# yjxiong/action-detection

Hardware: AMD Instinct MI355X
Metric: proposals/sec (9-seg BNInception SSN fwd+bwd) (higher is better)
Workload: dtype f32

## Files before the change

action-detection_amd/csrc/wgrad_pl.hip:

```cpp
#include "planes.h"

#include <algorithm>
#include <cmath>
#include <cstdlib>
#include <map>
#include <mutex>
#include <vector>

namespace {

using namespace pl;

struct WgPlArgs {
    const void* g_hi;
    const void* g_lo;
    const void* x_hi;
    const void* x_lo;
    float* part;
    unsigned long long* trace;
    int dbg;
    const float* g_scale;
    const float* x_scale;
    int g_row_split, g_row_gap;
    int N, Cin, H, W;
// ... 215 lines not shown
        __builtin_amdgcn_sched_barrier(0);
        read_begin(st[1]);
        mfma(cur, ks + NSTAGE, st[0], nxt);
        ++ks;
        const uint32_t o = st[0];
#pragma unroll
        for (int i = 0; i + 1 < NSTAGE; ++i) st[i] = st[i + 1];
        st[NSTAGE - 1] = o;
    };
    trc.mark1(p);
    for (int t = 0; t < nks; t += 2) {
        half(fr0, fr1);
        half(fr1, fr0);
    }
    SSN_WAIT_LGKM0();
    SSN_WAIT_VMCNT(0);
    trc.mark2(p);

    const float inv = 1.f / (*p.g_scale * *p.x_scale);
    const int KK = p.kh * p.kw;
    float* out = p.part + (long)z * p.M * p.ldp;
#pragma unroll
    for (int j = 0; j < TC; ++j) {
        const int ci = c0 + (wc * TC + j) * 32 + li;
        if (ci >= p.Cin) continue;
#pragma unroll
        for (int i = 0; i < TM; ++i) {
#pragma unroll
            for (int r = 0; r < 16; ++r) {
                const int m = m0 + (wm * TM + i) * 32 + (r & 3) + 8 * (r >> 2) + 4 * lh;
                if (m < p.M) out[(long)m * p.ldp + ci * KK + (int)tap] = acc[i][j][r] * inv;
            }
        }
    }
    if (do_bias && li == 0) {
        const float ginv = 1.f / *p.g_scale;
#pragma unroll
        for (int i = 0; i < TM; ++i)
#pragma unroll
            for (int r = 0; r < 16; ++r) {
                const int m = m0 + (wm * TM + i) * 32 + (r & 3) + 8 * (r >> 2) + 4 * lh;
                if (m < p.M) out[(long)m * p.ldp + p.K] = accb[i][r] * ginv;
            }
    }
    trc.end(p);
}

template <int WM, int WC, int TM, int TC>
__global__ __launch_bounds__(256, (TM * TC >= 6) ? 1 : 2) void wgrad_pl_kernel(WgPlArgs p) {
    __shared__ __attribute__((aligned(1024))) uint32_t lds[wgpl_lds_dwords<WM, WC, TM, TC>()];
    wgrad_pl_body<WM, WC, TM, TC>(p, blockIdx.x, lds);
}

template <int TM, int TC, int XP>
constexpr int wgpl9_lds_bytes() {
    return 2 * ((2 * TM) * 2 * 4 * 1024 + (2 * TC) * 2 * XP * 1024);
}

template <int KK, int TM, int TC, int XP, int KG = 1, int KH = 3, int KW = 3, int PH = 1, int PW = 1>
__device__ __forceinline__ void wgrad_pl9_body(const WgPlArgs& p, const uint32_t bid, unsigned char* lds) {
    constexpr int NS = 64, KSC = NS / 16;
    constexpr int KSG = KSC / KG;
    static_assert(KK == 1 || KK == KH * KW, "1x1, or all taps of the window");
    static_assert((KSG * KK) % 2 == 0, "steps come in pairs");
    static_assert(KG == 1 || KG == 2, "one or two wave groups");
    static_assert(XP % KG == 0, "X pieces split evenly between the wave groups");
    constexpr int BM = 2 * TM * 32, BC = 2 * TC * 32;
    constexpr int FA = BM / 32, FB = BC / 32;
    constexpr int A_BYTES = FA * 2 * KSC * 1024;
    constexpr int X_BYTES = FB * 2 * XP * 1024;
    constexpr int STAGE = A_BYTES + X_BYTES;
    static_assert(2 * STAGE == wgpl9_lds_bytes<TM, TC, XP>(), "LDS size");

    const int tid = threadIdx.x;
    WgTrace trc;
    trc.begin(p);
    const int lane = tid & 63, wave8 = wave_uniform(tid >> 6);
    const int wave = wave8 & 3, grp = wave8 >> 2;
    const int wm = wave >> 1, wc = wave & 1;
    const int li = lane & 31, lh = lane >> 5;

    const uint32_t tiles = (uint32_t)p.n_mtiles * (uint32_t)p.n_ctiles;
    const uint32_t logical = xcd_remap(bid, tiles * (uint32_t)p.splits);
    uint32_t z, tile, mt, ct;
    fd_divmod(logical, p.div_tiles, z, tile);
    fd_divmod(tile, p.div_ct, mt, ct);
    const int m0 = (int)mt * BM, c0 = (int)ct * BC;
    constexpr int BH = KK > 1 ? (PH > KH - 1 - PH ? PH : KH - 1 - PH) : 0, BW = KK > 1 ? (PW > KW - 1 - PW ? PW : KW - 1 - PW) : 0;
    const int Wp = p.W + BW, SP = (p.H + BH) * Wp;
    const int D = KK > 1 ? PH * Wp + PW : 0;
    const uint32_t T = (uint32_t)p.N * (uint32_t)SP;

    const int op = wave >> 1, plane = wave & 1;
    const void *xh = p.x_hi, *xl = p.x_lo, *gh = p.g_hi, *gl = p.g_lo;
    const uint32_t xbytes = p.x_bytes, gbytes = p.g_bytes, xgrp = p.x_grp_bytes, ggrp = p.g_grp_bytes, ximg = p.x_img_bytes, gimg = p.g_img_bytes;
    const __amdgpu_buffer_rsrc_t rsrc = op ? pl_rsrc(plane ? xl : xh, xbytes) : pl_rsrc(plane ? gl : gh, gbytes);
    const uint32_t grp_bytes = op ? xgrp : ggrp;
    const uint32_t img_bytes = op ? ximg : gimg;
    const int dsl = lane >> 2;
    const uint32_t lane_grp = (uint32_t)(lane & 3) * grp_bytes;
    constexpr int NF = FA > FB ? FA : FB;
    uint32_t frag_so[NF];
#pragma unroll
    for (int f = 0; f < NF; ++f) {
        const int ch = (op ? c0 : m0) + f * 32;
        const int gap = (!op && ch >= p.g_row_split) ? p.g_row_gap : 0;
        frag_so[f] = (uint32_t)((ch + gap) / 8) * grp_bytes;
    }
    const int ck_begin = (int)z * p.ksteps_per_split;
    const int total_ck = (int)((T + NS - 1) / NS);
    int ck_end = ck_begin + p.ksteps_per_split;
    if (ck_end > total_ck) ck_end = total_ck;

    constexpr int NPMAX = (XP > KSC ? XP : KSC) / KG;
    const int npieces = wave_uniform(op ? XP / KG : KSC / KG);
    const int lane_slot0 = (op ? -D : 0) + dsl;
    const uint32_t adv_img = (uint32_t)(NS / SP) * img_bytes, adv_u = (uint32_t)(NS % SP);
    uint32_t pu[NPMAX], pn[NPMAX];
#pragma unroll
    for (int q = 0; q < NPMAX; ++q) {
        const int sl = ck_begin * NS + lane_slot0 + (q * KG + grp) * 16;
        uint32_t n, u;
        fd_divmod((uint32_t)(sl < 0 ? sl + SP : sl), p.div_hw, n, u);
        pu[q] = u;
        pn[q] = (n - (sl < 0 ? 1u : 0u)) * img_bytes;
    }
    auto issue_piece = [&](int ck, int buf, int q) {
        if (q >= npieces || (WG_DBG(4) && ck > ck_begin)) return;
        const int sg = q * KG + grp;
        const int sl = ck * NS + lane_slot0 + sg * 16;
        const uint32_t hp = __umulhi(pu[q], p.magic_wp), wp = pu[q] - hp * (uint32_t)Wp;
        const bool real = ck < ck_end && (uint32_t)sl < T && hp >= (uint32_t)BH && wp >= (uint32_t)BW && !WG_DBG(1);
        const uint32_t vo = real ? pn[q] + ((hp - BH) * (uint32_t)p.W + (wp - BW)) * 16u + lane_grp : PL_OOB;
        unsigned char* base = lds + buf * STAGE;
        if (op == 0) {
#pragma unroll
            for (int f = 0; f < FA; ++f)
                WG_DMA_B128(rsrc, reinterpret_cast<uint32_t*>(base + ((f * 2 + plane) * KSC + sg) * 1024), vo, frag_so[f]);
        } else {
#pragma unroll
            for (int f = 0; f < FB; ++f)
                WG_DMA_B128(rsrc, reinterpret_cast<uint32_t*>(base + A_BYTES + ((f * 2 + plane) * XP + sg) * 1024), vo, frag_so[f]);
        }
        uint32_t u = pu[q] + adv_u, im = pn[q] + adv_img;
        const bool wrap = u >= (uint32_t)SP;
        pu[q] = wrap ? u - (uint32_t)SP : u;
        pn[q] = wrap ? im + img_bytes : im;
    };

    f32x16 acc[KK][TM][TC];
    f32x16 accb[TM];
#pragma unroll
    for (int i = 0; i < TM; ++i) {
#pragma unroll
        for (int r = 0; r < 16; ++r) accb[i][r] = 0.f;
#pragma unroll
        for (int t = 0; t < KK; ++t)
#pragma unroll
            for (int j = 0; j < TC; ++j)
#pragma unroll
                for (int r = 0; r < 16; ++r) acc[t][i][j][r] = 0.f;
    }
    const bool do_bias = wave_uniform((ct == 0 && wc == 0) ? 1 : 0) != 0;

    const int l16 = lane & 15, sg16 = (lane >> 4) & 1;
    const int lane_rd = (8 * lh + (l16 >> 2)) * 64 + sg16 * 32 + (l16 & 3) * 8;
    int tapoff[KK];
#pragma unroll
    for (int t = 0; t < KK; ++t) tapoff[t] = KK > 1 ? (D + (t / KW - PH) * Wp + (t % KW - PW)) * 64 : 0;
    const f16x8 ones = __builtin_bit_cast(f16x8, u32x4{0x3C003C00u, 0x3C003C00u, 0x3C003C00u, 0x3C003C00u});

#define WG_RD_FRAG(dst_, base_, imm_)                                                \
    do {                                                                             \
        u32x2 r0_, r1_;                                                              \
        SSN_DS_READ_TR16_B64_AT(r0_, base_, imm_);                                   \
        SSN_DS_READ_TR16_B64_AT(r1_, base_, (imm_) + 256);                           \
        dst_ = __builtin_bit_cast(f16x8, u32x4{r0_[0], r0_[1], r1_[0], r1_[1]});     \
    } while (0)

#pragma unroll
    for (int q = 0; q < NPMAX; ++q) issue_piece(ck_begin, 0, q);
    int buf = 0;
    trc.mark1(p);
    for (int ck = ck_begin; ck < ck_end; ++ck) {
        SSN_WAIT_VMCNT(0);
        __builtin_amdgcn_s_barrier();
        const unsigned char* ab = lds + buf * STAGE + lane_rd + grp * (KSG * 1024) + wm * (TM * 2 * KSC * 1024);
        const unsigned char* xb = lds + buf * STAGE + lane_rd + grp * (KSG * 1024) + A_BYTES + wc * (TC * 2 * XP * 1024);
        constexpr int NSTEP = KSG * KK, NPAIR = NSTEP / 2;
        static_assert(NSTEP % 2 == 0, "steps come in pairs");
        constexpr int NA = KK == 1 ? 4 : 2;
        f16x8 af[NA][2][TM], bf[4][2][TC];
        auto read_b = [&](int step, int set) {
            const int ks = step / KK, t = step % KK;
            const unsigned char* xt = xb + tapoff[t];
#pragma unroll
            for (int pn_ = 0; pn_ < 2; ++pn_)
#pragma unroll
                for (int j = 0; j < TC; ++j) WG_RD_FRAG(bf[set][pn_][j], xt, (j * 2 + pn_) * XP * 1024 + ks * 1024);
        };
        auto read_a = [&](int ks, int set) {
#pragma unroll
            for (int pn_ = 0; pn_ < 2; ++pn_)
#pragma unroll
                for (int i = 0; i < TM; ++i) WG_RD_FRAG(af[set][pn_][i], ab, ((i * 2 + pn_) * KSC + ks) * 1024);
        };
        read_a(0, 0);
        if (KK == 1) read_a(1, 1);
        read_b(0, 0);
        read_b(1, 1);
#pragma unroll
        for (int pr = 0; pr < NPAIR; ++pr) {
            const int s0 = 2 * pr, s1 = s0 + 1;
            const int ks0 = s0 / KK, t0 = s0 % KK, ks1 = s1 / KK, t1 = s1 % KK;
            SSN_WAIT_LGKM0();
            __builtin_amdgcn_sched_barrier(0);
            if (KK == 1) {
                if (ks0 + 2 < KSG) read_a(ks0 + 2, (ks0 + 2) % NA);
                if (ks1 + 2 < KSG) read_a(ks1 + 2, (ks1 + 2) % NA);
            } else {
                if (t0 == 1 && ks0 + 1 < KSG) read_a(ks0 + 1, (ks0 + 1) % NA);
                if (t1 == 1 && ks1 + 1 < KSG) read_a(ks1 + 1, (ks1 + 1) % NA);
            }
            if (s0 + 2 < NSTEP && !(WG_DBG(2) && (s0 + 2) % 3)) read_b(s0 + 2, (s0 + 2) % 4);
            if (s1 + 2 < NSTEP && !(WG_DBG(2) && (s1 + 2) % 3)) read_b(s1 + 2, (s1 + 2) % 4);
            constexpr int PPP = (NPMAX + 5) / 6;
#pragma unroll
            for (int e = 0; e < PPP; ++e)
                if (pr * PPP + e < NPMAX) issue_piece(ck + 1, buf ^ 1, pr * PPP + e);
            constexpr int PA[3] = {1, 0, 0};
            constexpr int PB[3] = {0, 0, 1};
#pragma unroll
            for (int c = 0; c < 3; ++c)
#pragma unroll
                for (int i = 0; i < TM; ++i)
#pragma unroll
                    for (int j = 0; j < TC; ++j) {
                        acc[t0][i][j] = __builtin_amdgcn_mfma_f32_32x32x16_f16(af[ks0 % NA][PA[c]][i], bf[s0 % 4][PB[c]][j], acc[t0][i][j],
                                                                               0, 0, 0);
                        acc[t1][i][j] = __builtin_amdgcn_mfma_f32_32x32x16_f16(af[ks1 % NA][PA[c]][i], bf[s1 % 4][PB[c]][j], acc[t1][i][j],
                                                                               0, 0, 0);
                    }
            if (do_bias) {
#pragma unroll
                for (int e = 0; e < 2; ++e) {
                    const int ks = e ? ks1 : ks0, t = e ? t1 : t0;
                    if (t != KK - 1) continue;
#pragma unroll
                    for (int i = 0; i < TM; ++i) {
                        accb[i] = __builtin_amdgcn_mfma_f32_32x32x16_f16(af[ks % NA][0][i], ones, accb[i], 0, 0, 0);
                        accb[i] = __builtin_amdgcn_mfma_f32_32x32x16_f16(af[ks % NA][1][i], ones, accb[i], 0, 0, 0);
                    }
                }
            }
        }
        if (NPMAX > NPAIR * ((NPMAX + 5) / 6)) {
#pragma unroll
            for (int q = NPAIR * ((NPMAX + 5) / 6); q < NPMAX; ++q) issue_piece(ck + 1, buf ^ 1, q);
        }
        buf ^= 1;
    }
    SSN_WAIT_VMCNT(0);
    trc.mark2(p);

    const float inv = 1.f / (*p.g_scale * *p.x_scale);
    float* out = p.part + ((long)z * KG + grp) * p.M * p.ldp;
#pragma unroll
    for (int j = 0; j < TC; ++j) {
        const int ci = c0 + (wc * TC + j) * 32 + li;
        if (ci >= p.Cin) continue;
#pragma unroll
        for (int i = 0; i < TM; ++i)
#pragma unroll
            for (int r = 0; r < 16; ++r) {
                const int m = m0 + (wm * TM + i) * 32 + (r & 3) + 8 * (r >> 2) + 4 * lh;
                if (m < p.M) {
#pragma unroll
                    for (int t = 0; t < KK; ++t) out[(long)m * p.ldp + t * p.Cin + ci] = acc[t][i][j][r] * inv;
                }
            }
    }
    if (do_bias && li == 0) {
        const float ginv = 1.f / *p.g_scale;
#pragma unroll
        for (int i = 0; i < TM; ++i)
#pragma unroll
            for (int r = 0; r < 16; ++r) {
                const int m = m0 + (wm * TM + i) * 32 + (r & 3) + 8 * (r >> 2) + 4 * lh;
                if (m < p.M) out[(long)m * p.ldp + p.K] = accb[i][r] * ginv;
            }
    }
    trc.end(p);
}

template <int KK, int TM, int TC, int XP, int KG = 1>
__global__ __launch_bounds__(256 * KG, (KG > 1 || KK * TM * TC >= 18 || TM * TC >= 4) ? 1 : 2) void wgrad_pl9_kernel(WgPlArgs p) {
    __shared__ __attribute__((aligned(1024))) unsigned char lds[wgpl9_lds_bytes<TM, TC, XP>()];
    wgrad_pl9_body<KK, TM, TC, XP, KG>(p, blockIdx.x, lds);
}


constexpr int WGG_MAX = 96;
constexpr int WGG_WRITE = 12;
struct WgGroupEntry {
    WgPlArgs a;
    int variant;
    uint32_t nblk;
};
struct WgGroupIndex {
    int count;
    int blk0[WGG_MAX + 1];
};
struct WgGroupChunk {
    WgGroupEntry e[WGG_WRITE];
    int count;
};
__global__ __launch_bounds__(64) void wgrad_group_write_kernel(WgGroupChunk c, WgGroupEntry* table, int first) {
    if ((int)threadIdx.x < c.count) table[first + threadIdx.x] = c.e[threadIdx.x];
}
__device__ __forceinline__ int group_problem_of_block(const WgGroupIndex& ix, int b) {
    int lo = 0, hi = ix.count - 1;
    while (lo < hi) {
        const int mid = (lo + hi + 1) >> 1;
        if (ix.blk0[mid] <= b) lo = mid; else hi = mid - 1;
    }
    return wave_uniform(lo);
}

template <int XP, int KG, int KH = 3, int KW = 3>
__global__ __launch_bounds__(256 * KG, KG > 1 ? 1 : 2) void wgrad_group9_kernel(const WgGroupEntry* __restrict__ table, WgGroupIndex ix) {
    __shared__ __attribute__((aligned(1024))) unsigned char lds[wgpl9_lds_bytes<1, 1, XP>()];
    const int e = group_problem_of_block(ix, (int)blockIdx.x);
    const uint32_t bid = blockIdx.x - (uint32_t)ix.blk0[e];
    const auto* ent = SSN_CONST_PTR(WgGroupEntry, table) + e;
    if (bid >= ent->nblk) return;
    const WgPlArgs p = ent->a;
    wgrad_pl9_body<KH * KW, 1, 1, XP, KG, KH, KW, KH / 2, KW / 2>(p, bid, lds);
}

constexpr int WGG1_LDS = 65536;
static_assert(wgpl_lds_dwords<2, 2, 2, 2>() * 4 <= WGG1_LDS && wgpl_lds_dwords<1, 4, 3, 1>() * 4 <= WGG1_LDS &&
              wgpl_lds_dwords<2, 2, 1, 1>() * 4 <= WGG1_LDS && wgpl9_lds_bytes<1, 1, 4>() <= WGG1_LDS, "group LDS");
__global__ __launch_bounds__(256, 2) void wgrad_group1_kernel(const WgGroupEntry* __restrict__ table, WgGroupIndex ix) {
    __shared__ __attribute__((aligned(1024))) unsigned char lds[WGG1_LDS];
    const int e = group_problem_of_block(ix, (int)blockIdx.x);
    const uint32_t bid = blockIdx.x - (uint32_t)ix.blk0[e];
    const auto* ent = SSN_CONST_PTR(WgGroupEntry, table) + e;
    if (bid >= ent->nblk) return;
    const WgPlArgs p = ent->a;
    switch (wave_uniform(ent->variant)) {
        case 0: wgrad_pl_body<2, 2, 2, 2>(p, bid, reinterpret_cast<uint32_t*>(lds)); break;
        case 1: wgrad_pl_body<1, 4, 3, 1>(p, bid, reinterpret_cast<uint32_t*>(lds)); break;
        case 2: wgrad_pl_body<2, 2, 1, 1>(p, bid, reinterpret_cast<uint32_t*>(lds)); break;
        default: wgrad_pl9_body<1, 1, 1, 4>(p, bid, lds); break;
    }
}

constexpr int STEM_NS = 128;
constexpr int STEM_DA = 256;
constexpr int STEM_EA = 128;
constexpr int STEM_RING = 1024;
constexpr int STEM_MAX_W = 114;
constexpr int STEM_LDS = 2 * (2 * 2 * 8 * 1024) + 2 * STEM_RING * 32;
inline bool stem_layer(int kh, int kw, int stride, int pad_h, int pad_w, int H, int W, int Ho, int Wo) {
    return kh == 4 && kw == 4 && stride == 1 && pad_h == 2 && pad_w == 2 && Ho == H && Wo == W && W <= STEM_MAX_W;
}
__device__ __forceinline__ void wgrad_stem_body(const WgPlArgs& p, const uint32_t bid, unsigned char* lds) {
    constexpr int NS = STEM_NS, KSC = NS / 16, KG = 2, KSG = KSC / KG;
    constexpr int A_BYTES = 2 * 2 * KSC * 1024;
    constexpr int RING_BYTES = STEM_RING * 32;
    constexpr uint32_t RMASK = STEM_RING - 1;
    static_assert(2 * A_BYTES + 2 * RING_BYTES == STEM_LDS, "LDS size");
    static_assert(STEM_DA >= 2 * (STEM_MAX_W + 2) + 2 && STEM_EA >= STEM_MAX_W + 3 && STEM_DA + 2 * NS + STEM_EA <= STEM_RING, "window");
    unsigned char* const xring = lds + 2 * A_BYTES;

    const int tid = threadIdx.x;
    const int lane = tid & 63, wave8 = wave_uniform(tid >> 6);
    const int wave = wave8 & 3, grp = wave8 >> 2;
    const int wm = wave & 1, wc = wave >> 1;
    const int li = lane & 31, lh = lane >> 5;

    const uint32_t tiles = (uint32_t)p.n_mtiles * (uint32_t)p.n_ctiles;
    const uint32_t logical = xcd_remap(bid, tiles * (uint32_t)p.splits);
    uint32_t z, tile, mt, sub;
    fd_divmod(logical, p.div_tiles, z, tile);
    fd_divmod(tile, p.div_ct, mt, sub);
    const int m0 = (int)mt * 64, c0 = (int)sub * 16;
    const int Wp = p.W + 2, SP = (p.H + 2) * Wp;
    const int T = p.N * SP;

// ... 98 lines not shown
            constexpr int PB[3] = {0, 0, 1};
#pragma unroll
            for (int c = 0; c < 3; ++c)
#pragma unroll
                for (int i = 0; i < 4; ++i)
                    acc[i] = __builtin_amdgcn_mfma_f32_32x32x16_f16(af[ks & 1][PA[c]], bf[ks & 1][i][PB[c]], acc[i], 0, 0, 0);
            if (do_bias) {
                accb = __builtin_amdgcn_mfma_f32_32x32x16_f16(af[ks & 1][0], ones, accb, 0, 0, 0);
                accb = __builtin_amdgcn_mfma_f32_32x32x16_f16(af[ks & 1][1], ones, accb, 0, 0, 0);
            }
        }
        buf ^= 1;
    }
    SSN_WAIT_VMCNT(0);

    const float inv = 1.f / (*p.g_scale * *p.x_scale);
    float* out = p.part + ((long)z * KG + grp) * p.M * p.ldp;
    const int ci = c0 + (li & 15);
    if (ci < p.Cin) {
#pragma unroll
        for (int i = 0; i < 4; ++i) {
            const int pi = wc * 4 + i;
            const int t = ((pi >> 2) + 2 * (li >> 4)) * 4 + (pi & 3);
#pragma unroll
            for (int r = 0; r < 16; ++r) {
                const int m = m0 + wm * 32 + (r & 3) + 8 * (r >> 2) + 4 * lh;
                if (m < p.M) out[(long)m * p.ldp + t * p.Cin + ci] = acc[i][r] * inv;
            }
        }
    }
    if (do_bias && li == 0) {
        const float ginv = 1.f / *p.g_scale;
#pragma unroll
        for (int r = 0; r < 16; ++r) {
            const int m = m0 + wm * 32 + (r & 3) + 8 * (r >> 2) + 4 * lh;
            if (m < p.M) out[(long)m * p.ldp + p.K] = accb[r] * ginv;
        }
    }
}

__global__ __launch_bounds__(512, 1) void wgrad_group_stem_kernel(const WgGroupEntry* __restrict__ table, WgGroupIndex ix) {
    __shared__ __attribute__((aligned(1024))) unsigned char lds[STEM_LDS];
    const int e = group_problem_of_block(ix, (int)blockIdx.x);
    const uint32_t bid = blockIdx.x - (uint32_t)ix.blk0[e];
    const auto* ent = SSN_CONST_PTR(WgGroupEntry, table) + e;
    if (bid >= ent->nblk) return;
    const WgPlArgs p = ent->a;
    wgrad_stem_body(p, bid, lds);
}

#undef WG_DMA_B128
#undef WG_RD_FRAG

template <int KK, int TM, int TC, int XP, int KG = 1>
int launch_wgpl9(WgPlArgs& a, hipStream_t stream) {
    constexpr int BM = 2 * TM * 32, BC = 2 * TC * 32;
    a.n_mtiles = (a.M + BM - 1) / BM;
    a.n_ctiles = (a.Cin + BC - 1) / BC;
    const unsigned tiles = (unsigned)a.n_mtiles * (unsigned)a.n_ctiles;
    a.div_tiles = make_fastdiv(tiles);
    a.div_ct = make_fastdiv((uint32_t)a.n_ctiles);
    a.magic_wp = 0xFFFFFFFFu / (uint32_t)(a.W + (KK > 1 ? 1 : 0)) + 1u;
    hipLaunchKernelGGL((wgrad_pl9_kernel<KK, TM, TC, XP, KG>), dim3(tiles * (unsigned)a.splits), dim3(256 * KG), 0, stream, a);
    SSN_CHECK_LAUNCH("wgrad_pl9");
    return SSN_OK;
}

constexpr int N9 = 4;
const int k9BM[N9] = {64, 128, 64, 64};
const int k9BC[N9] = {64, 64, 128, 64};
const int k9Occ[N9] = {1, 1, 1, 1};
const int k9KG[N9] = {1, 1, 1, 2};

template <int XP>
int launch_wgpl9_xp(WgPlArgs& a, int cfg, hipStream_t stream) {
    switch (cfg) {
        case 0: return launch_wgpl9<9, 1, 1, XP>(a, stream);
        case 1: return launch_wgpl9<9, 2, 1, XP>(a, stream);
        case 2: return launch_wgpl9<9, 1, 2, XP>(a, stream);
        case 3: return launch_wgpl9<9, 1, 1, XP, 2>(a, stream);
    }
    ssn_set_error("conv_wgrad_pl (nine taps): unknown tile config %d", cfg);
    return SSN_ERR_ARG;
}
int xp_for(int W) { return (64 + 2 * (W + 2) + 15) / 16; }
int launch_wgpl9_tile(WgPlArgs& a, int cfg, hipStream_t stream) {
    const int xp = xp_for(a.W);
    if (xp <= 6) return launch_wgpl9_xp<6>(a, cfg, stream);
    if (xp <= 8) return launch_wgpl9_xp<8>(a, cfg, stream);
    return cfg == 3 ? launch_wgpl9<9, 1, 1, 12, 2>(a, stream) : launch_wgpl9<9, 1, 1, 12>(a, stream);
}
constexpr int N1 = 4;
const int k1BM[N1] = {64, 128, 64, 128};
const int k1BC[N1] = {64, 64, 128, 128};
const int k1Occ[N1] = {2, 1, 1, 1};
int launch_wgpl1_tile(WgPlArgs& a, int cfg, hipStream_t stream) {
    switch (cfg) {
        case 0: return launch_wgpl9<1, 1, 1, 4>(a, stream);
        case 1: return launch_wgpl9<1, 2, 1, 4>(a, stream);
        case 2: return launch_wgpl9<1, 1, 2, 4>(a, stream);
        case 3: return launch_wgpl9<1, 2, 2, 4>(a, stream);
    }
    ssn_set_error("conv_wgrad_pl (chunked 1x1): unknown tile config %d", cfg);
    return SSN_ERR_ARG;
}
void plan1(int M, int Cin, long slots, int cfg, int* splits, int* chunks_per_split) {
    const long tiles = (long)((M + k1BM[cfg] - 1) / k1BM[cfg]) * ((Cin + k1BC[cfg] - 1) / k1BC[cfg]);
    const long chunks = (slots + 63) / 64;
    plan_split_k(tiles, chunks, k1Occ[cfg], 4, 2, 0.005 + (double)M * Cin * 1.7e-6, splits, chunks_per_split);
}
bool chunked_1x1_layer(int kh, int kw, int stride, int pad_h, int pad_w) {
    return kh == 1 && kw == 1 && stride == 1 && pad_h == 0 && pad_w == 0;
}

int pick_tile9(int M, int Cin, int W) {
    if (xp_for(W) > 8) return 0;
    double best = 1e300;
    int bc = 0;
    for (int c = 0; c < 3; ++c) {
        const double padded = (double)((M + k9BM[c] - 1) / k9BM[c]) * k9BM[c] * (double)((Cin + k9BC[c] - 1) / k9BC[c]) * k9BC[c];
        const double small = c == 0 ? 1.1 : 1.0;
        if (padded * small < best) {
            best = padded * small;
            bc = c;
        }
    }
    return bc;
}
void plan9(int M, int Cin, long slots, int cfg, int W, int* splits, int* chunks_per_split) {
    const long tiles = (long)((M + k9BM[cfg] - 1) / k9BM[cfg]) * ((Cin + k9BC[cfg] - 1) / k9BC[cfg]);
    const long chunks = (slots + 63) / 64;
    const int occ = (cfg == 0 && xp_for(W) <= 6) ? 2 : k9Occ[cfg];
    plan_split_k(tiles, chunks, occ, 4, 2, 0.005 + (double)M * Cin * 9 * 1.7e-6, splits, chunks_per_split);
}
bool nine_tap_layer(int kh, int kw, int stride, int pad_h, int pad_w, int H, int W, int Ho, int Wo) {
    return kh == 3 && kw == 3 && stride == 1 && pad_h == 1 && pad_w == 1 && Ho == H && Wo == W && W + 2 <= 58;
}

template <int WM, int WC, int TM, int TC>
int launch_wgpl(WgPlArgs& a, hipStream_t stream) {
// ... 231 lines not shown
                }
            }
        }
    }
    it.variant = v;
    a.n_mtiles = (a.M + kG1BM[v] - 1) / kG1BM[v];
    a.n_ctiles = (a.Cin + kG1BC[v] - 1) / kG1BC[v];
    a.div_ct = make_fastdiv((uint32_t)a.n_ctiles);
    it.chunked = v == 3;
    if (it.chunked) {
        it.tiles = (long)a.n_mtiles * a.n_ctiles;
        it.units = ((long)a.P + 63) / 64;
        it.unit_cost = 4 * 3.0 * (kG1BM[v] / 64) * (kG1BC[v] / 64);
        a.magic_wp = 0xFFFFFFFFu / (uint32_t)a.W + 1u;
        a.div_hw = make_fastdiv((uint32_t)(a.H * a.W));
        a.div_w = make_fastdiv((uint32_t)a.W);
    } else {
        const int KK = a.kh * a.kw;
        it.tiles = (long)a.n_mtiles * a.n_ctiles * KK;
        it.units = ((long)a.P + 15) / 16;
        it.unit_cost = 3.0 * (kG1BM[v] / 32) * (kG1BC[v] / 32) / 4;
        a.div_kk = make_fastdiv((uint32_t)KK);
    }
    a.div_tiles = make_fastdiv((uint32_t)it.tiles);
    return SSN_OK;
}
void plan_group(std::vector<WgGroupItem*>& fam, int slots, double fixed_cost, int min_units, bool even_units) {
    double work = 0;
    for (WgGroupItem* it : fam) work += (double)it->tiles * (double)it->units * it->unit_cost;
    double target = std::sqrt(2.0 * fixed_cost * work / slots);
    if (target < fixed_cost) target = fixed_cost;
    for (WgGroupItem* it : fam) {
        long per = (long)(target / it->unit_cost + 0.5);
        const long floor_units = (it->family >= WGF_1 && it->chunked) ? (min_units + 3) / 4 : min_units;
        if (per < floor_units) per = floor_units;
        if (it->pin > 0) per = it->pin;
        if (per > it->units) per = it->units;
        long splits = (it->units + per - 1) / per;
        per = (it->units + splits - 1) / splits;
        if (even_units && !it->chunked && (per & 1)) ++per;
        splits = (it->units + per - 1) / per;
        it->a.splits = (int)splits;
        it->a.ksteps_per_split = (int)per;
    }
}

bool group1_interleave() {
    static const bool on = [] {
        const char* e = std::getenv("SSN_WGRAD_INTERLEAVE");
        return !(e && e[0] == '0');
    }();
    return on;
}

}

extern "C" void ssn_conv_wgrad_pl_debug_trace(unsigned long long* buf) { g_wg_trace = buf; }
extern "C" void ssn_conv_wgrad_pl_debug_flags(int flags) { g_wg_dbg = flags; }

extern "C" int ssn_wgrad_reduce(const float* part, float* dw, float* db, int M, int K, int splits, hipStream_t stream);
extern "C" int ssn_wgrad_reduce_taps(const float* part, float* dw, float* db, int M, int K, int splits, int taps, hipStream_t stream);

extern "C" int ssn_conv_wgrad_pl_tiles(void) { return NCFG; }

extern "C" long ssn_conv_wgrad_pl_workspace_bytes(int N, int Cin, int Cout, int Ho, int Wo, int kh, int kw, int tile_cfg) {
    if (tile_cfg >= 200) {
        int s1, c1;
        plan1(Cout, Cin, (long)N * Ho * Wo, (tile_cfg - 200) < N1 ? tile_cfg - 200 : 0, &s1, &c1);
        return (long)s1 * Cout * ((long)Cin + 1) * (long)sizeof(float);
    }
    if (tile_cfg >= 100 || (tile_cfg < 0 && kh == 3 && kw == 3)) {
        int c9 = tile_cfg >= 100 ? tile_cfg - 100 : pick_tile9(Cout, Cin, Wo);
        if (c9 >= N9 || (xp_for(Wo) > 8 && c9 != 3)) c9 = 0;
        int splits9, cps9;
        plan9(Cout, Cin, (long)N * (Ho + 1) * (Wo + 1), c9, Wo, &splits9, &cps9);
        const long need9 = (long)splits9 * k9KG[c9] * Cout * ((long)Cin * 9 + 1) * (long)sizeof(float);
        if (tile_cfg >= 100) return need9;
        const int cfg1 = fix_cfg(-1, Cout, Cin);
        int s1, k1;
        plan(Cout, Cin, 9, (long)N * Ho * Wo, cfg1, &s1, &k1);
        const long need1 = (long)s1 * Cout * ((long)Cin * 9 + 1) * (long)sizeof(float);
        return need9 > need1 ? need9 : need1;
    }
    const int cfg = fix_cfg(tile_cfg, Cout, Cin);
    int splits, kps;
    plan(Cout, Cin, kh * kw, (long)N * Ho * Wo, cfg, &splits, &kps);
    return (long)splits * Cout * ((long)Cin * kh * kw + 1) * (long)sizeof(float);
}

namespace {
int plan_group_all(int count, const int* shape, const long* groups, const void* const* g_hi, const void* const* g_lo,
                   const void* const* x_hi, const void* const* x_lo, float* const* dw, float* const* db, const float* const* g_scale,
                   const float* const* x_scale, std::vector<WgGroupItem>& items, long* ws_total) {
    items.resize((size_t)count);
    static const float one = 1.f;
    for (int i = 0; i < count; ++i) {
        const int* sh = shape + (size_t)i * 16;
        WgGroupItem& it = items[(size_t)i];
        const void* dummy = &one;
        int rc = fill_wgpl(it.a, g_hi ? g_hi[i] : dummy, g_lo ? g_lo[i] : dummy, x_hi ? x_hi[i] : dummy, x_lo ? x_lo[i] : dummy, sh[0], sh[1],
                           sh[2], sh[3], groups[i * 2], sh[4], sh[5], sh[6], groups[i * 2 + 1], sh[7], sh[8], sh[9], sh[10], sh[11],
                           g_scale ? g_scale[i] : &one, x_scale ? x_scale[i] : &one, sh[12], sh[13]);
        if (rc != SSN_OK) return rc;
        it.dw = dw ? dw[i] : nullptr;
        it.db = db ? db[i] : nullptr;
        SSN_CHECK_ARG(sh[15] >= 0, "conv wgrad pl group: problem %d: units per split %d", i, sh[15]);
        it.pin = sh[15];
        rc = classify_group(it, sh[14]);
        if (rc != SSN_OK) return rc;
    }
    for (int f = 0; f < WGF_COUNT; ++f) {
        std::vector<WgGroupItem*> fam;
        for (WgGroupItem& it : items)
            if (it.family == f) fam.push_back(&it);
        if (fam.empty()) continue;
        if (f == WGF_1)
            plan_group(fam, 512, g_group_fixed[1], g_group_min_units[1], true);
        else
            plan_group(fam, (f == WGF_9_XP6 || f == WGF_7_ROW) ? 512 : 256, g_group_fixed[0], g_group_min_units[0], false);
    }
    long off = 0;
    for (WgGroupItem& it : items) {
        it.ws_off = off;
        off += ((long)it.a.splits * it.kg * it.a.M * it.a.ldp * (long)sizeof(float) + 1023) / 1024 * 1024;
    }
    *ws_total = off;
// ... 105 lines not shown
            };
            std::stable_sort(fam.begin(), fam.end(), [&](const WgGroupItem* x, const WgGroupItem* y) { return bytes_per_mac(x) > bytes_per_mac(y); });
            std::vector<WgGroupItem*> dealt;
            for (size_t lo = 0, hi = fam.size(); lo < hi;) {
                dealt.push_back(fam[lo++]);
                if (lo < hi) dealt.push_back(fam[--hi]);
            }
            fam.swap(dealt);
        }
        for (size_t base = 0; base < fam.size(); base += WGG_MAX) {
            const int n = (int)std::min<size_t>(WGG_MAX, fam.size() - base);
            Launch L;
            L.family = f;
            L.first = first;
            L.items.assign(fam.begin() + (long)base, fam.begin() + (long)base + n);
            L.slab_bytes = 0;
            for (const WgGroupItem* it : L.items) L.slab_bytes += (long)it->a.splits * it->kg * it->a.M * it->a.ldp * (long)sizeof(float);
            launches.push_back(std::move(L));
            first += n;
        }
    }
    if (per_family)
        std::stable_sort(launches.begin(), launches.end(), [](const Launch& x, const Launch& y) { return x.slab_bytes > y.slab_bytes; });

    int fan = n_lanes;
#if defined(__HIP__)
    WgLaneEvents* ev = fan > 0 ? wgrad_lane_events(stream) : nullptr;
    if (!ev) fan = 0;
#else
    SSN_CHECK_ARG(n_lanes == 0, "conv wgrad pl group: the host build has no streams");
#endif

    auto write_table = [&](const Launch& L, WgGroupIndex& ix) -> long {
        const int n = (int)L.items.size();
        ix.count = n;
        long blocks = 0;
        for (int c0 = 0; c0 < n; c0 += WGG_WRITE) {
            WgGroupChunk ch;
            ch.count = std::min(WGG_WRITE, n - c0);
            for (int j = 0; j < ch.count; ++j) {
                WgGroupItem& it = *L.items[(size_t)(c0 + j)];
                it.a.part = reinterpret_cast<float*>(static_cast<char*>(workspace) + it.ws_off);
                ch.e[j].a = it.a;
                ch.e[j].variant = it.variant;
                ch.e[j].nblk = (uint32_t)(it.tiles * it.a.splits);
                ix.blk0[c0 + j] = (int)blocks;
                blocks += (it.tiles * it.a.splits + 7) / 8 * 8;
            }
            hipLaunchKernelGGL(wgrad_group_write_kernel, dim3(1), dim3(64), 0, stream, ch, dev, L.first + c0);
        }
        for (int j = n; j <= WGG_MAX; ++j) ix.blk0[j] = (int)blocks;
        return blocks;
    };
    auto launch_family = [&](const Launch& L, const WgGroupIndex& ix, long blocks, hipStream_t s) {
        const WgGroupEntry* tab = dev + L.first;
        switch (L.family) {
            case WGF_9_XP6: hipLaunchKernelGGL((wgrad_group9_kernel<6, 1>), dim3((unsigned)blocks), dim3(256), 0, s, tab, ix); break;
            case WGF_9_XP8: hipLaunchKernelGGL((wgrad_group9_kernel<8, 2>), dim3((unsigned)blocks), dim3(512), 0, s, tab, ix); break;
            case WGF_9_XP12: hipLaunchKernelGGL((wgrad_group9_kernel<12, 2>), dim3((unsigned)blocks), dim3(512), 0, s, tab, ix); break;
            case WGF_STEM: hipLaunchKernelGGL(wgrad_group_stem_kernel, dim3((unsigned)blocks), dim3(512), 0, s, tab, ix); break;
            case WGF_7_ROW: hipLaunchKernelGGL((wgrad_group9_kernel<6, 1, 1, 7>), dim3((unsigned)blocks), dim3(256), 0, s, tab, ix); break;
            case WGF_7_COL: hipLaunchKernelGGL((wgrad_group9_kernel<12, 2, 7, 1>), dim3((unsigned)blocks), dim3(512), 0, s, tab, ix); break;
            default: hipLaunchKernelGGL(wgrad_group1_kernel, dim3((unsigned)blocks), dim3(256), 0, s, tab, ix); break;
        }
    };
    auto reduce = [&](const std::vector<const WgGroupItem*>& its, hipStream_t s) -> int {
        const size_t n = its.size();
        std::vector<const float*> parts(n);
        std::vector<float*> dws(n), dbs(n);
        std::vector<int> Ms(n), Ks(n), sp(n), tp(n);
        for (size_t i = 0; i < n; ++i) {
            const WgGroupItem& it = *its[i];
            parts[i] = reinterpret_cast<const float*>(static_cast<char*>(workspace) + it.ws_off);
            dws[i] = it.dw;
            dbs[i] = it.db;
            Ms[i] = it.a.M;
            Ks[i] = it.a.K;
            sp[i] = it.a.splits * it.kg;
            tp[i] = it.taps;
        }
        return ssn_wgrad_reduce_multi((int)n, parts.data(), dws.data(), dbs.data(), Ms.data(), Ks.data(), sp.data(), tp.data(), s);
    };

    std::vector<WgGroupIndex> index(launches.size());
    std::vector<long> grid(launches.size());
    if (fan > 0) {
        for (size_t k = 0; k < launches.size(); ++k) {
            grid[k] = write_table(launches[k], index[k]);
            SSN_CHECK_ARG(grid[k] < (1l << 31), "conv wgrad pl group: too many blocks");
        }
        SSN_CHECK_LAUNCH("conv_wgrad_pl_group");
    }
#if defined(__HIP__)
    if (fan > 0) {
        bool ok = hipEventRecord(ev->fork, stream) == hipSuccess;
        for (int k = 0; k < fan && ok; ++k) ok = hipStreamWaitEvent(lanes[k], ev->fork, 0) == hipSuccess;
        if (!ok) {
            ssn_set_error("conv wgrad pl group: fork of the side streams failed: %s", hipGetErrorString(hipGetLastError()));
            return SSN_ERR_LAUNCH;
        }
    }
#endif
    for (size_t k = 0; k < launches.size(); ++k) {
        const Launch& L = launches[k];
        hipStream_t s = fan > 0 ? lanes[k % (size_t)fan] : stream;
        if (fan == 0) {
            grid[k] = write_table(L, index[k]);
            SSN_CHECK_ARG(grid[k] < (1l << 31), "conv wgrad pl group: too many blocks");
        }
        launch_family(L, index[k], grid[k], s);
        if (per_family) {
            SSN_CHECK_LAUNCH("conv_wgrad_pl_group");
// ... 25 lines not shown

extern "C" int ssn_conv_wgrad_pl_group(int count, const void* const* g_hi, const void* const* g_lo, const void* const* x_hi,
                                       const void* const* x_lo, float* const* dw, float* const* db, const int* shape,
                                       const long* groups, const float* const* g_scale, const float* const* x_scale, void* workspace,
                                       long ws_bytes, void* table, long table_bytes, hipStream_t stream) {
    return wgrad_group_run(count, g_hi, g_lo, x_hi, x_lo, dw, db, shape, groups, g_scale, x_scale, workspace, ws_bytes, table,
                           table_bytes, stream, false, nullptr, 0, true);
}

extern "C" int ssn_conv_wgrad_pl_group_lanes(int count, const void* const* g_hi, const void* const* g_lo, const void* const* x_hi,
                                             const void* const* x_lo, float* const* dw, float* const* db, const int* shape,
                                             const long* groups, const float* const* g_scale, const float* const* x_scale,
                                             void* workspace, long ws_bytes, void* table, long table_bytes, hipStream_t stream,
                                             const hipStream_t* lanes, int n_lanes, int join) {
    return wgrad_group_run(count, g_hi, g_lo, x_hi, x_lo, dw, db, shape, groups, g_scale, x_scale, workspace, ws_bytes, table,
                           table_bytes, stream, true, lanes, n_lanes, join != 0);
}

extern "C" int ssn_conv_wgrad_pl(const void* g_hi, const void* g_lo, const void* x_hi, const void* x_lo, float* dw, float* db,
                                 int N, int Cin, int H, int W, long x_img_groups, int Cout, int Ho, int Wo, long g_img_groups,
                                 int kh, int kw, int stride, int pad_h, int pad_w, void* workspace, long ws_bytes, int tile_cfg,
                                 const float* g_scale, const float* x_scale, int g_row_split, int g_row_gap,
                                 int* deferred_reduce, hipStream_t stream) {
    SSN_CHECK_ARG(dw && workspace, "conv wgrad pl: null pointer");
    WgPlArgs a;
    const int rcf = fill_wgpl(a, g_hi, g_lo, x_hi, x_lo, N, Cin, H, W, x_img_groups, Cout, Ho, Wo, g_img_groups, kh, kw, stride, pad_h, pad_w,
                              g_scale, x_scale, g_row_split, g_row_gap);
    if (rcf != SSN_OK) return rcf;
    a.part = (float*)workspace;
    if (tile_cfg >= 200) {
        SSN_CHECK_ARG(chunked_1x1_layer(kh, kw, stride, pad_h, pad_w) && tile_cfg - 200 < N1,
                      "conv wgrad pl: the chunked kernel (tile %d) takes 1x1 / stride-1 layers only", tile_cfg);
        const int c1 = tile_cfg - 200;
        plan1(Cout, Cin, a.P, c1, &a.splits, &a.ksteps_per_split);
        const long need1 = (long)a.splits * Cout * a.ldp * (long)sizeof(float);
        if (ws_bytes < need1) {
            ssn_set_error("conv wgrad pl: workspace %ld < %ld bytes", ws_bytes, need1);
            return SSN_ERR_WORKSPACE;
        }
        a.div_hw = make_fastdiv((uint32_t)(H * W));
        a.div_w = make_fastdiv((uint32_t)W);
        const int rc1 = launch_wgpl1_tile(a, c1, stream);
        if (rc1 != SSN_OK) return rc1;
        if (deferred_reduce) {
            deferred_reduce[0] = a.splits;
            deferred_reduce[1] = 1;
            return SSN_OK;
        }
        return ssn_wgrad_reduce(a.part, dw, db, Cout, a.K, a.splits, stream);
    }
    if ((tile_cfg >= 100 || tile_cfg < 0) && nine_tap_layer(kh, kw, stride, pad_h, pad_w, H, W, Ho, Wo)) {
        int c9 = tile_cfg >= 100 ? tile_cfg - 100 : pick_tile9(Cout, Cin, W);
        SSN_CHECK_ARG(c9 < N9, "conv wgrad pl: unknown nine-tap tile %d", c9);
        if (xp_for(W) > 8 && c9 != 3) c9 = 0;
        plan9(Cout, Cin, (long)N * (H + 1) * (W + 1), c9, W, &a.splits, &a.ksteps_per_split);
        const long need9 = (long)a.splits * k9KG[c9] * Cout * a.ldp * (long)sizeof(float);
        if (ws_bytes < need9) {
            ssn_set_error("conv wgrad pl: workspace %ld < %ld bytes", ws_bytes, need9);
            return SSN_ERR_WORKSPACE;
        }
        a.div_hw = make_fastdiv((uint32_t)((H + 1) * (W + 1)));
        a.div_w = make_fastdiv((uint32_t)(W + 1));
        const int rc9 = launch_wgpl9_tile(a, c9, stream);
        if (rc9 != SSN_OK) return rc9;
        if (deferred_reduce) {
            deferred_reduce[0] = a.splits * k9KG[c9];
            deferred_reduce[1] = 9;
            return SSN_OK;
        }
        return ssn_wgrad_reduce_taps(a.part, dw, db, Cout, a.K, a.splits * k9KG[c9], 9, stream);
    }
    SSN_CHECK_ARG(tile_cfg < 100, "conv wgrad pl: the nine-tap kernel takes 3x3 / stride 1 / pad 1 layers only");
    const int cfg = fix_cfg(tile_cfg, Cout, Cin);
    plan(Cout, Cin, kh * kw, a.P, cfg, &a.splits, &a.ksteps_per_split);
    const long need = (long)a.splits * Cout * a.ldp * (long)sizeof(float);
    if (ws_bytes < need) {
        ssn_set_error("conv wgrad pl: workspace %ld < %ld bytes", ws_bytes, need);
        return SSN_ERR_WORKSPACE;
    }
    const int rc = launch_wgpl_tile(a, cfg, stream);
    if (rc != SSN_OK) return rc;
    if (deferred_reduce) {
        deferred_reduce[0] = a.splits;
        deferred_reduce[1] = 1;
        return SSN_OK;
    }
    return ssn_wgrad_reduce(a.part, dw, db, Cout, a.K, a.splits, stream);
}
```

Measured before the change: 2343.

## Add X ring buffer to nine-tap wgrad to reload only new slots per chunk

Adds a ring-buffer form of the nine-tap weight-gradient kernel. The X operand lives in a circular LDS ring, so each chunk issues DMA only for its 64 new slots instead of reloading the whole overlapping window (halo included). Reads wrap addresses with a mask. The ring form is enabled by default for the grouped XP12 family, is available for XP8 through an env var, and is exposed as a new tile config 104. The cost is extra address arithmetic on each B-fragment read and a different LDS footprint.

```diff
diff --git a/action-detection_amd/csrc/wgrad_pl.hip b/action-detection_amd/csrc/wgrad_pl.hip
--- a/action-detection_amd/csrc/wgrad_pl.hip
+++ b/action-detection_amd/csrc/wgrad_pl.hip
@@ -291,12 +291,13 @@
     wgrad_pl_body<WM, WC, TM, TC>(p, blockIdx.x, lds);
 }
 
-template <int TM, int TC, int XP>
+constexpr int WG9_RING = 256;
+template <int TM, int TC, int XP, bool RING = false>
 constexpr int wgpl9_lds_bytes() {
-    return 2 * ((2 * TM) * 2 * 4 * 1024 + (2 * TC) * 2 * XP * 1024);
-}
-
-template <int KK, int TM, int TC, int XP, int KG = 1, int KH = 3, int KW = 3, int PH = 1, int PW = 1>
+    return RING ? 2 * (2 * TM) * 2 * 4 * 1024 + (2 * TC) * 2 * WG9_RING * 64 : 2 * ((2 * TM) * 2 * 4 * 1024 + (2 * TC) * 2 * XP * 1024);
+}
+
+template <int KK, int TM, int TC, int XP, int KG = 1, int KH = 3, int KW = 3, int PH = 1, int PW = 1, bool RING = false>
 __device__ __forceinline__ void wgrad_pl9_body(const WgPlArgs& p, const uint32_t bid, unsigned char* lds) {
     constexpr int NS = 64, KSC = NS / 16;
     constexpr int KSG = KSC / KG;
@@ -304,12 +305,18 @@
     static_assert((KSG * KK) % 2 == 0, "steps come in pairs");
     static_assert(KG == 1 || KG == 2, "one or two wave groups");
     static_assert(XP % KG == 0, "X pieces split evenly between the wave groups");
+    static_assert(!RING || (KK > 1 && KG == 2 && XP > KSC && 16 * XP + NS <= WG9_RING && (WG9_RING & (WG9_RING - 1)) == 0),
+                  "ring form: multi-tap, two wave groups, the window and the 64 new slots of the next chunk fit the ring side by side");
     constexpr int BM = 2 * TM * 32, BC = 2 * TC * 32;
     constexpr int FA = BM / 32, FB = BC / 32;
     constexpr int A_BYTES = FA * 2 * KSC * 1024;
     constexpr int X_BYTES = FB * 2 * XP * 1024;
-    constexpr int STAGE = A_BYTES + X_BYTES;
-    static_assert(2 * STAGE == wgpl9_lds_bytes<TM, TC, XP>(), "LDS size");
+    constexpr int STAGE = RING ? A_BYTES : A_BYTES + X_BYTES;
+    constexpr int RING_BYTES = WG9_RING * 64;
+    constexpr uint32_t RMASK = RING_BYTES - 1;
+    static_assert((RING ? 2 * A_BYTES + FB * 2 * RING_BYTES : 2 * STAGE) == wgpl9_lds_bytes<TM, TC, XP, RING>(), "LDS size");
+    static_assert(!RING || 2 * A_BYTES + (2 * TC - 1) * RING_BYTES < 65536, "ring form: the rings of a wave within reach of a read's immediate");
+    unsigned char* const xring = lds + 2 * A_BYTES;
 
     const int tid = threadIdx.x;
     WgTrace trc;
@@ -364,9 +371,11 @@
         pu[q] = u;
         pn[q] = (n - (sl < 0 ? 1u : 0u)) * img_bytes;
     }
-    auto issue_piece = [&](int ck, int buf, int q) {
+    constexpr int NSTEADY = RING ? KSC / KG : NPMAX;
+    const int sgoff = RING ? wave_uniform(op ? XP - KSC : 0) : 0;
+    auto issue_piece = [&](int ck, int buf, int q, int sg0) {
         if (q >= npieces || (WG_DBG(4) && ck > ck_begin)) return;
-        const int sg = q * KG + grp;
+        const int sg = q * KG + grp + sg0;
         const int sl = ck * NS + lane_slot0 + sg * 16;
         const uint32_t hp = __umulhi(pu[q], p.magic_wp), wp = pu[q] - hp * (uint32_t)Wp;
         const bool real = ck < ck_end && (uint32_t)sl < T && hp >= (uint32_t)BH && wp >= (uint32_t)BW && !WG_DBG(1);
@@ -376,6 +385,11 @@
 #pragma unroll
             for (int f = 0; f < FA; ++f)
                 WG_DMA_B128(rsrc, reinterpret_cast<uint32_t*>(base + ((f * 2 + plane) * KSC + sg) * 1024), vo, frag_so[f]);
+        } else if (RING) {
+            const uint32_t rowb = (uint32_t)((ck * NS + sg * 16) * 64) & RMASK;
+#pragma unroll
+            for (int f = 0; f < FB; ++f)
+                WG_DMA_B128(rsrc, reinterpret_cast<uint32_t*>(xring + (f * 2 + plane) * RING_BYTES + rowb), vo, frag_so[f]);
         } else {
 #pragma unroll
             for (int f = 0; f < FB; ++f)
@@ -418,7 +432,15 @@
     } while (0)
 
 #pragma unroll
-    for (int q = 0; q < NPMAX; ++q) issue_piece(ck_begin, 0, q);
+    for (int q = 0; q < NPMAX; ++q) issue_piece(ck_begin, 0, q, 0);
+    if constexpr (RING) {
+#pragma unroll
+        for (int e = 0; e < NSTEADY; ++e) {
+            const uint32_t ux = pu[XP / KG - NSTEADY + e], ug = pu[e], nx = pn[XP / KG - NSTEADY + e], ng = pn[e];
+            pu[e] = op ? ux : ug;
+            pn[e] = op ? nx : ng;
+        }
+    }
     int buf = 0;
     trc.mark1(p);
     for (int ck = ck_begin; ck < ck_end; ++ck) {
@@ -426,17 +448,33 @@
         __builtin_amdgcn_s_barrier();
         const unsigned char* ab = lds + buf * STAGE + lane_rd + grp * (KSG * 1024) + wm * (TM * 2 * KSC * 1024);
         const unsigned char* xb = lds + buf * STAGE + lane_rd + grp * (KSG * 1024) + A_BYTES + wc * (TC * 2 * XP * 1024);
+        constexpr uint32_t XWRAP = ~(uint32_t)RING_BYTES;
+        const uint32_t xr0 = ((uint32_t)(ck * (NS * 64) + grp * (KSG * 1024) + lane_rd) & RMASK) + (uint32_t)(wc * (TC * 2 * RING_BYTES));
         constexpr int NSTEP = KSG * KK, NPAIR = NSTEP / 2;
         static_assert(NSTEP % 2 == 0, "steps come in pairs");
         constexpr int NA = KK == 1 ? 4 : 2;
         f16x8 af[NA][2][TM], bf[4][2][TC];
         auto read_b = [&](int step, int set) {
             const int ks = step / KK, t = step % KK;
-            const unsigned char* xt = xb + tapoff[t];
-#pragma unroll
-            for (int pn_ = 0; pn_ < 2; ++pn_)
-#pragma unroll
-                for (int j = 0; j < TC; ++j) WG_RD_FRAG(bf[set][pn_][j], xt, (j * 2 + pn_) * XP * 1024 + ks * 1024);
+            if constexpr (RING) {
+                const uint32_t o = xr0 + (uint32_t)tapoff[t] + (uint32_t)(ks * 1024);
+                const unsigned char *q0 = lds + (o & XWRAP), *q1 = lds + ((o + 256u) & XWRAP);
+#pragma unroll
+                for (int pn_ = 0; pn_ < 2; ++pn_)
+#pragma unroll
+                    for (int j = 0; j < TC; ++j) {
+                        u32x2 v0, v1;
+                        SSN_DS_READ_TR16_B64_AT(v0, q0, 2 * A_BYTES + (j * 2 + pn_) * RING_BYTES);
+                        SSN_DS_READ_TR16_B64_AT(v1, q1, 2 * A_BYTES + (j * 2 + pn_) * RING_BYTES);
+                        bf[set][pn_][j] = __builtin_bit_cast(f16x8, u32x4{v0[0], v0[1], v1[0], v1[1]});
+                    }
+            } else {
+                const unsigned char* xt = xb + tapoff[t];
+#pragma unroll
+                for (int pn_ = 0; pn_ < 2; ++pn_)
+#pragma unroll
+                    for (int j = 0; j < TC; ++j) WG_RD_FRAG(bf[set][pn_][j], xt, (j * 2 + pn_) * XP * 1024 + ks * 1024);
+            }
         };
         auto read_a = [&](int ks, int set) {
 #pragma unroll
@@ -463,10 +501,10 @@
             }
             if (s0 + 2 < NSTEP && !(WG_DBG(2) && (s0 + 2) % 3)) read_b(s0 + 2, (s0 + 2) % 4);
             if (s1 + 2 < NSTEP && !(WG_DBG(2) && (s1 + 2) % 3)) read_b(s1 + 2, (s1 + 2) % 4);
-            constexpr int PPP = (NPMAX + 5) / 6;
+            constexpr int PPP = (NSTEADY + 5) / 6;
 #pragma unroll
             for (int e = 0; e < PPP; ++e)
-                if (pr * PPP + e < NPMAX) issue_piece(ck + 1, buf ^ 1, pr * PPP + e);
+                if (pr * PPP + e < NSTEADY) issue_piece(ck + 1, buf ^ 1, pr * PPP + e, sgoff);
             constexpr int PA[3] = {1, 0, 0};
             constexpr int PB[3] = {0, 0, 1};
 #pragma unroll
@@ -493,9 +531,9 @@
                 }
             }
         }
-        if (NPMAX > NPAIR * ((NPMAX + 5) / 6)) {
-#pragma unroll
-            for (int q = NPAIR * ((NPMAX + 5) / 6); q < NPMAX; ++q) issue_piece(ck + 1, buf ^ 1, q);
+        if (NSTEADY > NPAIR * ((NSTEADY + 5) / 6)) {
+#pragma unroll
+            for (int q = NPAIR * ((NSTEADY + 5) / 6); q < NSTEADY; ++q) issue_piece(ck + 1, buf ^ 1, q, sgoff);
         }
         buf ^= 1;
     }
@@ -532,10 +570,10 @@
     trc.end(p);
 }
 
-template <int KK, int TM, int TC, int XP, int KG = 1>
+template <int KK, int TM, int TC, int XP, int KG = 1, bool RING = false>
 __global__ __launch_bounds__(256 * KG, (KG > 1 || KK * TM * TC >= 18 || TM * TC >= 4) ? 1 : 2) void wgrad_pl9_kernel(WgPlArgs p) {
-    __shared__ __attribute__((aligned(1024))) unsigned char lds[wgpl9_lds_bytes<TM, TC, XP>()];
-    wgrad_pl9_body<KK, TM, TC, XP, KG>(p, blockIdx.x, lds);
+    __shared__ __attribute__((aligned(1024))) unsigned char lds[wgpl9_lds_bytes<TM, TC, XP, RING>()];
+    wgrad_pl9_body<KK, TM, TC, XP, KG, 3, 3, 1, 1, RING>(p, blockIdx.x, lds);
 }
 
 
@@ -566,15 +604,16 @@
     return wave_uniform(lo);
 }
 
-template <int XP, int KG, int KH = 3, int KW = 3>
+template <int XP, int KG, int KH = 3, int KW = 3, bool RING = false>
 __global__ __launch_bounds__(256 * KG, KG > 1 ? 1 : 2) void wgrad_group9_kernel(const WgGroupEntry* __restrict__ table, WgGroupIndex ix) {
-    __shared__ __attribute__((aligned(1024))) unsigned char lds[wgpl9_lds_bytes<1, 1, XP>()];
+    __shared__ __attribute__((aligned(1024))) unsigned char lds[wgpl9_lds_bytes<1, 1, XP, RING>()];
+    static_assert(wgpl9_lds_bytes<1, 1, XP, RING>() * (KG > 1 ? 1 : 2) <= 160 * 1024, "group LDS");
     const int e = group_problem_of_block(ix, (int)blockIdx.x);
     const uint32_t bid = blockIdx.x - (uint32_t)ix.blk0[e];
     const auto* ent = SSN_CONST_PTR(WgGroupEntry, table) + e;
     if (bid >= ent->nblk) return;
     const WgPlArgs p = ent->a;
-    wgrad_pl9_body<KH * KW, 1, 1, XP, KG, KH, KW, KH / 2, KW / 2>(p, bid, lds);
+    wgrad_pl9_body<KH * KW, 1, 1, XP, KG, KH, KW, KH / 2, KW / 2, RING>(p, bid, lds);
 }
 
 constexpr int WGG1_LDS = 65536;
@@ -779,7 +818,7 @@
 #undef WG_DMA_B128
 #undef WG_RD_FRAG
 
-template <int KK, int TM, int TC, int XP, int KG = 1>
+template <int KK, int TM, int TC, int XP, int KG = 1, bool RING = false>
 int launch_wgpl9(WgPlArgs& a, hipStream_t stream) {
     constexpr int BM = 2 * TM * 32, BC = 2 * TC * 32;
     a.n_mtiles = (a.M + BM - 1) / BM;
@@ -788,16 +827,16 @@
     a.div_tiles = make_fastdiv(tiles);
     a.div_ct = make_fastdiv((uint32_t)a.n_ctiles);
     a.magic_wp = 0xFFFFFFFFu / (uint32_t)(a.W + (KK > 1 ? 1 : 0)) + 1u;
-    hipLaunchKernelGGL((wgrad_pl9_kernel<KK, TM, TC, XP, KG>), dim3(tiles * (unsigned)a.splits), dim3(256 * KG), 0, stream, a);
+    hipLaunchKernelGGL((wgrad_pl9_kernel<KK, TM, TC, XP, KG, RING>), dim3(tiles * (unsigned)a.splits), dim3(256 * KG), 0, stream, a);
     SSN_CHECK_LAUNCH("wgrad_pl9");
     return SSN_OK;
 }
 
-constexpr int N9 = 4;
-const int k9BM[N9] = {64, 128, 64, 64};
-const int k9BC[N9] = {64, 64, 128, 64};
-const int k9Occ[N9] = {1, 1, 1, 1};
-const int k9KG[N9] = {1, 1, 1, 2};
+constexpr int N9 = 5;
+const int k9BM[N9] = {64, 128, 64, 64, 64};
+const int k9BC[N9] = {64, 64, 128, 64, 64};
+const int k9Occ[N9] = {1, 1, 1, 1, 1};
+const int k9KG[N9] = {1, 1, 1, 2, 2};
 
 template <int XP>
 int launch_wgpl9_xp(WgPlArgs& a, int cfg, hipStream_t stream) {
@@ -813,6 +852,10 @@
 int xp_for(int W) { return (64 + 2 * (W + 2) + 15) / 16; }
 int launch_wgpl9_tile(WgPlArgs& a, int cfg, hipStream_t stream) {
     const int xp = xp_for(a.W);
+    if (cfg == 4) {
+        SSN_CHECK_ARG(xp > 6, "conv wgrad pl: nine-tap tile 104 (X ring) takes rows of > 14 pixels only (W = %d)", a.W);
+        return xp <= 8 ? launch_wgpl9<9, 1, 1, 8, 2, true>(a, stream) : launch_wgpl9<9, 1, 1, 12, 2, true>(a, stream);
+    }
     if (xp <= 6) return launch_wgpl9_xp<6>(a, cfg, stream);
     if (xp <= 8) return launch_wgpl9_xp<8>(a, cfg, stream);
     return cfg == 3 ? launch_wgpl9<9, 1, 1, 12, 2>(a, stream) : launch_wgpl9<9, 1, 1, 12>(a, stream);
@@ -1150,6 +1193,10 @@
     }();
     return on;
 }
+int group9_ring() {
+    const char* e = std::getenv("SSN_WGRAD_RING");
+    return (e && e[0] >= '0' && e[0] <= '2') ? e[0] - '0' : 1;
+}
 
 }
 
@@ -1169,7 +1216,7 @@
     }
     if (tile_cfg >= 100 || (tile_cfg < 0 && kh == 3 && kw == 3)) {
         int c9 = tile_cfg >= 100 ? tile_cfg - 100 : pick_tile9(Cout, Cin, Wo);
-        if (c9 >= N9 || (xp_for(Wo) > 8 && c9 != 3)) c9 = 0;
+        if (c9 >= N9 || (xp_for(Wo) > 8 && c9 < 3)) c9 = 0;
         int splits9, cps9;
         plan9(Cout, Cin, (long)N * (Ho + 1) * (Wo + 1), c9, Wo, &splits9, &cps9);
         const long need9 = (long)splits9 * k9KG[c9] * Cout * ((long)Cin * 9 + 1) * (long)sizeof(float);
@@ -1381,12 +1428,23 @@
         for (int j = n; j <= WGG_MAX; ++j) ix.blk0[j] = (int)blocks;
         return blocks;
     };
+    const int ring_level = group9_ring();
     auto launch_family = [&](const Launch& L, const WgGroupIndex& ix, long blocks, hipStream_t s) {
         const WgGroupEntry* tab = dev + L.first;
         switch (L.family) {
             case WGF_9_XP6: hipLaunchKernelGGL((wgrad_group9_kernel<6, 1>), dim3((unsigned)blocks), dim3(256), 0, s, tab, ix); break;
-            case WGF_9_XP8: hipLaunchKernelGGL((wgrad_group9_kernel<8, 2>), dim3((unsigned)blocks), dim3(512), 0, s, tab, ix); break;
-            case WGF_9_XP12: hipLaunchKernelGGL((wgrad_group9_kernel<12, 2>), dim3((unsigned)blocks), dim3(512), 0, s, tab, ix); break;
+            case WGF_9_XP8:
+                if (ring_level >= 2)
+                    hipLaunchKernelGGL((wgrad_group9_kernel<8, 2, 3, 3, true>), dim3((unsigned)blocks), dim3(512), 0, s, tab, ix);
+                else
+                    hipLaunchKernelGGL((wgrad_group9_kernel<8, 2>), dim3((unsigned)blocks), dim3(512), 0, s, tab, ix);
+                break;
+            case WGF_9_XP12:
+                if (ring_level >= 1)
+                    hipLaunchKernelGGL((wgrad_group9_kernel<12, 2, 3, 3, true>), dim3((unsigned)blocks), dim3(512), 0, s, tab, ix);
+                else
+                    hipLaunchKernelGGL((wgrad_group9_kernel<12, 2>), dim3((unsigned)blocks), dim3(512), 0, s, tab, ix);
+                break;
             case WGF_STEM: hipLaunchKernelGGL(wgrad_group_stem_kernel, dim3((unsigned)blocks), dim3(512), 0, s, tab, ix); break;
             case WGF_7_ROW: hipLaunchKernelGGL((wgrad_group9_kernel<6, 1, 1, 7>), dim3((unsigned)blocks), dim3(256), 0, s, tab, ix); break;
             case WGF_7_COL: hipLaunchKernelGGL((wgrad_group9_kernel<12, 2, 7, 1>), dim3((unsigned)blocks), dim3(512), 0, s, tab, ix); break;
@@ -1518,7 +1576,8 @@
     if ((tile_cfg >= 100 || tile_cfg < 0) && nine_tap_layer(kh, kw, stride, pad_h, pad_w, H, W, Ho, Wo)) {
         int c9 = tile_cfg >= 100 ? tile_cfg - 100 : pick_tile9(Cout, Cin, W);
         SSN_CHECK_ARG(c9 < N9, "conv wgrad pl: unknown nine-tap tile %d", c9);
-        if (xp_for(W) > 8 && c9 != 3) c9 = 0;
+        if (xp_for(W) > 8 && c9 < 3) c9 = 0;
+        SSN_CHECK_ARG(c9 != 4 || xp_for(W) > 6, "conv wgrad pl: nine-tap tile 104 (X ring) takes rows of > 14 pixels only (W = %d)", W);
         plan9(Cout, Cin, (long)N * (H + 1) * (W + 1), c9, W, &a.splits, &a.ksteps_per_split);
         const long need9 = (long)a.splits * k9KG[c9] * Cout * a.ldp * (long)sizeof(float);
         if (ws_bytes < need9) {
```

New measurement: 2357 (median of 6 runs). No clear change (+0.6%).
